# addtt/ladder-vae-pytorch

Measured on AMD Instinct MI355X. Metric: training images/sec (ELBO step: fwd+bwd+Adamax), higher is better.
Workload: dtype f32; 1 GPU; CIFAR10-shaped 15-layer LVAE (BASELINE configs[2]): 32x32x3, zdims 32x15, 4 blocks/layer, 64 filters, gated+skip, DMoL-10, dropout 0.2, free bits 1.0; batch_per_gpu=256, global_batch=256, parallelism=dp1, hip_graph=True

## Files before the change

### include/lvae_hip.h

```cpp
#ifndef LVAE_HIP_H
#define LVAE_HIP_H

#include <stddef.h>
#include <stdint.h>

#ifdef __cplusplus
extern "C" {
#endif

#define LVAE_ABI_VERSION 17

#define LVAE_EINVAL (-1)
#define LVAE_EALIGN (-2)
#define LVAE_EWORKSPACE (-3)

enum { LVAE_STATS_BN_FWD = 0, LVAE_STATS_BN_BWD = 1 };
enum { LVAE_PREC_F32 = 0, LVAE_PREC_BF16 = 1 };
enum { LVAE_DT_F32 = 0, LVAE_DT_BF16 = 1 };
enum {
  LVAE_FORM_AUTO = 0,
  LVAE_FORM_F32_MFMA = 1,
  LVAE_FORM_SIX_PRODUCT = 2,
  LVAE_FORM_SIX_PRODUCT_DIRECT = 3
};
enum { LVAE_ACT_NONE = 0, LVAE_ACT_ELU = 1, LVAE_ACT_RELU = 2, LVAE_ACT_LEAKYRELU = 3, LVAE_ACT_SELU = 4 };

enum {
  LVAE_GATHER_CONV = 0,
  LVAE_GATHER_TRANSPOSED = 1
};

int lvae_abi_version(void);
const char* lvae_last_error(void);

typedef struct lvae_bn_fold {
  const float* parts;
  int32_t rows;
  int64_t M;
  const float* gamma;
  const float* beta;
  float eps, momentum;
  float* running_mean;
  float* running_var;
  float* coef_out;
} lvae_bn_fold;

typedef struct lvae_conv_desc {
  const float* x;
  const float* x2;
  int32_t C1, C2;
  const float* w;
  int64_t w_stap, w_sk, w_sn;
  const float* bias;
  const float* in_scale;
  const float* in_shift;
  int32_t in_act;
  const float* out_scale;
  int32_t out_act;
  float* y;
  int32_t N, H, W, OH, OW, Cout;
  int32_t KH, KW, stride, pad;
  int32_t gather;
  int32_t precision;
  void* workspace;
  int64_t workspace_bytes;
  int32_t workspace_ready;
  float* stats_out;
  const float* stats_pivot;
  int32_t stats_mode;
  int32_t stats_act;
  const float* stats_x;
  const struct lvae_bn_fold* in_fold;
  int32_t form;
  uint8_t x_dtype;
  uint8_t y_dtype;
  uint8_t stats_x_dtype;
  uint8_t reserved_;
} lvae_conv_desc;

size_t lvae_conv2d_workspace(const lvae_conv_desc* d);
int lvae_conv2d_f32(const lvae_conv_desc* d, void* stream);
int lvae_conv1x1_dgrad_cat_f32(const lvae_conv_desc* d, float* dx2, int32_t split, void* stream);
int32_t lvae_conv1x1_dgrad_cat_ok(const lvae_conv_desc* d, int32_t split);
enum {
  LVAE_VARIANT_DIRECT = 0,
  LVAE_VARIANT_POS = 2,
  LVAE_VARIANT_WINO_F32 = 3,
  LVAE_VARIANT_WINO_SIX = 4,
  LVAE_VARIANT_BF16_DIRECT = 5,
  LVAE_VARIANT_SIX_DIRECT = 6
};
int32_t lvae_conv2d_variant(const lvae_conv_desc* d);
int32_t lvae_resblock_bf16_storage(const lvae_conv_desc* d);
int lvae_conv2d_bf16(const lvae_conv_desc* d, void* stream);
int32_t lvae_conv2d_stats_rows(const lvae_conv_desc* d);
int32_t lvae_conv2d_folds_bn_finalize(const lvae_conv_desc* d);
int32_t lvae_conv2d_stats_buffer_rows(const lvae_conv_desc* d);

size_t lvae_conv2d_prepare_entry_bytes(void);
int lvae_conv2d_prepare_entry(const lvae_conv_desc* d, void* entry);
int lvae_conv2d_prepare_weights(const void* entries, int32_t n, int32_t max_cout, void* stream);

int lvae_conv1x1_gate_f32(const lvae_conv_desc* d, const float* res, int32_t act, float* out, void* stream);
int32_t lvae_conv1x1_gate_stats_rows(const lvae_conv_desc* d);
enum {
  LVAE_GATE_PERSISTENT = 1,
  LVAE_GATE_SINGLE_SHOT = 2
};
int32_t lvae_conv1x1_gate_variant(const lvae_conv_desc* d);
int lvae_conv1x1_gate_bwd_f32(const lvae_conv_desc* d, const float* dout, const float* ab, int32_t act, float* dab,
                              void* stream);
int32_t lvae_conv1x1_gate_bwd_ok(const lvae_conv_desc* d);

typedef struct lvae_bn_apply {
  const float* parts;
  int32_t rows;
  int32_t act;
  int64_t M;
  const float* coef;
  const float* dh;
  const float* x;
  const float* add;
  float* dgamma;
  float* dbeta;
  float* out;
  int32_t dh_bf16;
  int32_t reserved_;
  const float* drop;
} lvae_bn_apply;
size_t lvae_conv1x1_gate_bwd_wgrad_workspace(const lvae_conv_desc* d);
int32_t lvae_conv1x1_gate_bwd_wgrad_apply_ok(const lvae_conv_desc* d);
int lvae_conv1x1_gate_bwd_wgrad_f32(const lvae_conv_desc* d, const float* dout, const float* ab, const float* y, int32_t act,
                                    float* dw, int64_t dw_sk, int64_t dw_sn, float* db, void* workspace, size_t workspace_bytes,
                                    const lvae_bn_apply* ap, void* stream);

enum { LVAE_RB_PRO_AFFINE = 0, LVAE_RB_PRO_BN_APPLY = 1, LVAE_RB_PRO_GATE_BWD = 2 };
enum { LVAE_RB_EPI_PLAIN = 0, LVAE_RB_EPI_GATE = 1 };
typedef struct lvae_rb_ext {
  int32_t prologue, epilogue;
  const float* gate_w;
  int64_t gate_w_sk, gate_w_sn;
  void* gate_ws;
  int64_t gate_ws_bytes;
  int32_t gate_ws_ready;
  const float* gate_bias;
  int32_t act;
  const float* res;
  float* ab;
  float* out;
  float* out_stats;
  const float* out_stats_pivot;
  const float* dout;
  const float* ab_in;
  float* dab;
  const float* bwd_parts;
  int32_t bwd_rows;
  int32_t bwd_act;
  int64_t bwd_M;
  const float* bwd_coef;
  const float* bwd_x;
  float* dgamma;
  float* dbeta;
  const float* pro_drop;
  float* xt_out;
  const void* pf_ptr[2];
  int64_t pf_bytes[2];
  const float* ap_parts;
  int32_t ap_rows;
  int32_t ap_act;
  int64_t ap_M;
  const float* ap_coef;
  const float* ap_dh;
  const float* ap_x;
  const float* ap_add;
  float* ap_dgamma;
  float* ap_dbeta;
  float* ap_out;
} lvae_rb_ext;
size_t lvae_resblock_gate_workspace(const lvae_conv_desc* g);
int lvae_resblock_gate_prepare_entry(const lvae_conv_desc* g, void* entry);
int32_t lvae_resblock_conv_rows(const lvae_conv_desc* d);
int32_t lvae_resblock_conv_gate_rows(const lvae_conv_desc* d);
size_t lvae_resblock_conv_workspace(const lvae_conv_desc* d);
int lvae_resblock_conv_prepare_entry(const lvae_conv_desc* d, void* entry);
int lvae_resblock_conv_f32(const lvae_conv_desc* d, const lvae_rb_ext* ext, void* stream);

size_t lvae_conv2d_wgrad_workspace(const lvae_conv_desc* d);
int lvae_conv2d_wgrad_f32(const lvae_conv_desc* d, const float* dy, float* dw, float* db, void* workspace,
                          size_t workspace_bytes, void* stream);
int lvae_conv2d_wgrad_bf16(const lvae_conv_desc* d, const float* dy, float* dw, float* db, void* workspace, size_t workspace_bytes,
                           void* stream);
int32_t lvae_conv2d_wgrad_apply_ok(const lvae_conv_desc* d);
int lvae_conv2d_wgrad_apply_f32(const lvae_conv_desc* d, const lvae_bn_apply* ap, float* dw, float* db, void* workspace,
                                size_t workspace_bytes, void* stream);
enum {
  LVAE_WGRAD_VARIANT_GENERIC = 0,
  LVAE_WGRAD_VARIANT_IMG = 1,
  LVAE_WGRAD_VARIANT_BF16 = 2,
  LVAE_WGRAD_VARIANT_WINO = 3,
  LVAE_WGRAD_VARIANT_DIRECT_1X1 = 4,
  LVAE_WGRAD_VARIANT_TILE = 5,
  LVAE_WGRAD_VARIANT_THIN = 6
};
int32_t lvae_conv2d_wgrad_variant(const lvae_conv_desc* d);
size_t lvae_conv2d_wgrad_grouped_workspace(const lvae_conv_desc* descs, int32_t n);
int lvae_conv2d_wgrad_grouped_f32(const lvae_conv_desc* descs, const float* const* dy, float* const* dw, float* const* db,
                                  int32_t n, void* workspace, size_t workspace_bytes, void* stream);
int32_t lvae_conv2d_wgrad_grouped_schedule(const lvae_conv_desc* descs, int32_t n, int32_t* launch_of);

size_t lvae_bn_stats_workspace(int64_t M, int32_t C);
int lvae_bn_stats_f32(const float* x, int64_t M, int32_t C, const float* gamma, const float* beta, float eps,
                      float momentum, float* running_mean, float* running_var, float* scale, float* shift,
                      float* mean, float* rstd, void* workspace, size_t workspace_bytes, void* stream);
int lvae_bn_finalize_parts_f32(const float* parts, int32_t rows, int64_t M, int32_t C, const float* pivot, const float* gamma,
                               const float* beta, float eps, float momentum, float* running_mean, float* running_var,
                               float* scale, float* shift, float* mean, float* rstd, void* stream);
int lvae_bn_eval_coeffs_f32(int32_t C, const float* gamma, const float* beta, const float* running_mean,
                            const float* running_var, float eps, float* scale, float* shift, void* stream);

int lvae_affine_act_f32(const float* x, int64_t M, int32_t C, const float* scale, const float* shift, int32_t act,
                        const float* row_scale, int64_t rows_per_n, float* y, void* stream);

int lvae_affine_act_bwd_f32(const float* dh, const float* x, int64_t M, int32_t C, const float* scale,
                            const float* shift, int32_t act, int32_t bn_train, const float* mean, const float* rstd,
                            float* dgamma, float* dbeta, const float* drop, int64_t rows_per_n, const float* add,
                            float* dx, void* workspace, size_t workspace_bytes, void* stream);
int lvae_affine_act_bwd_parts_f32(const float* parts, int32_t rows, const float* dh, const float* x, int64_t M, int32_t C,
                                  const float* scale, const float* shift, int32_t act, const float* mean, const float* rstd,
                                  float* dgamma, float* dbeta, const float* drop, int64_t rows_per_n, const float* add,
                                  float* dx, void* workspace, size_t workspace_bytes, int32_t dtypes, void* stream);

int lvae_gate_fwd_f32(const float* ab, const float* res, int64_t M, int32_t C, int32_t act, float* out, void* stream);
int lvae_gate_bwd_f32(const float* dout, const float* ab, int64_t M, int32_t C, int32_t act, float* dab, void* stream);

int lvae_act_bwd_from_out_f32(const float* dy, const float* y, int64_t n, int32_t act, float* dx, void* stream);
int lvae_add_f32(const float* a, const float* b, int64_t n, float* out, void* stream);
int lvae_add3_f32(const float* a, const float* b, const float* c, int64_t n, float* out, void* stream);
int lvae_sum_of_row_means_f32(const float* x, int32_t L, int32_t N, float* out, void* stream);
int lvae_scale_rows_add_f32(const float* a, const float* row_scale, int64_t rows_per_n, int32_t C, const float* b,
                            int64_t M, float* out, void* stream);
int lvae_colsum_f32(const float* x, int64_t R, int64_t P, float* out, int32_t accumulate, void* stream);

int lvae_normal_stochastic_fwd_f32(const float* p, int32_t p_bcast, const float* q, const float* eps, int32_t N,
                                   int32_t HW, int32_t Z, int32_t mode, int32_t analytical_kl, float* z,
                                   float* logprob_p, float* logprob_q, float* kl_samplewise, float* kl_spatial,
// ... 121 lines not shown
```

### ladder-vae-pytorch_amd/_C.py

```python
import ctypes as C
import os

import torch

_HERE = os.path.dirname(os.path.abspath(__file__))
LIB_PATH = os.path.join(_HERE, 'liblvae_hip.so')

ACT = {None: 0, 'none': 0, 'elu': 1, 'relu': 2, 'leakyrelu': 3, 'selu': 4}
GATHER_CONV, GATHER_TRANSPOSED = 0, 1
PREC_F32, PREC_BF16 = 0, 1
DT_F32, DT_BF16 = 0, 1
VARIANT_DIRECT, VARIANT_POS, VARIANT_WINO_F32, VARIANT_WINO_SIX, VARIANT_BF16_DIRECT, VARIANT_SIX_DIRECT = 0, 2, 3, 4, 5, 6
GATE_PERSISTENT, GATE_SINGLE_SHOT = 1, 2
WGRAD_VARIANT_GENERIC, WGRAD_VARIANT_IMG, WGRAD_VARIANT_BF16, WGRAD_VARIANT_WINO, WGRAD_VARIANT_DIRECT_1X1, WGRAD_VARIANT_TILE, WGRAD_VARIANT_THIN = range(7)
FEED_U8, FEED_F32 = 0, 1
FORM_AUTO, FORM_F32_MFMA, FORM_SIX_PRODUCT, FORM_SIX_PRODUCT_DIRECT = 0, 1, 2, 3


class LvaeHipError(RuntimeError):
    pass


class ConvDesc(C.Structure):
    _fields_ = [
        ('x', C.c_void_p), ('x2', C.c_void_p), ('C1', C.c_int32), ('C2', C.c_int32),
        ('w', C.c_void_p), ('w_stap', C.c_int64), ('w_sk', C.c_int64), ('w_sn', C.c_int64),
        ('bias', C.c_void_p), ('in_scale', C.c_void_p), ('in_shift', C.c_void_p), ('in_act', C.c_int32),
        ('out_scale', C.c_void_p), ('out_act', C.c_int32), ('y', C.c_void_p),
        ('N', C.c_int32), ('H', C.c_int32), ('W', C.c_int32), ('OH', C.c_int32), ('OW', C.c_int32),
        ('Cout', C.c_int32), ('KH', C.c_int32), ('KW', C.c_int32), ('stride', C.c_int32), ('pad', C.c_int32),
        ('gather', C.c_int32), ('precision', C.c_int32), ('workspace', C.c_void_p), ('workspace_bytes', C.c_int64), ('workspace_ready', C.c_int32), ('stats_out', C.c_void_p), ('stats_pivot', C.c_void_p), ('stats_mode', C.c_int32), ('stats_act', C.c_int32),
        ('stats_x', C.c_void_p),
        ('in_fold', C.c_void_p),
        ('form', C.c_int32), ('x_dtype', C.c_uint8), ('y_dtype', C.c_uint8), ('stats_x_dtype', C.c_uint8), ('reserved_', C.c_uint8),
    ]


class BnFold(C.Structure):
    _fields_ = [('parts', C.c_void_p), ('rows', C.c_int32), ('M', C.c_int64), ('gamma', C.c_void_p), ('beta', C.c_void_p),
                ('eps', C.c_float), ('momentum', C.c_float), ('running_mean', C.c_void_p), ('running_var', C.c_void_p),
                ('coef_out', C.c_void_p)]


class BnApply(C.Structure):
    _fields_ = [('parts', C.c_void_p), ('rows', C.c_int32), ('act', C.c_int32), ('M', C.c_int64), ('coef', C.c_void_p), ('dh', C.c_void_p),
                ('x', C.c_void_p), ('add', C.c_void_p), ('dgamma', C.c_void_p), ('dbeta', C.c_void_p), ('out', C.c_void_p),
                ('dh_bf16', C.c_int32), ('reserved_', C.c_int32), ('drop', C.c_void_p)]


class RbExt(C.Structure):
    _fields_ = [('prologue', C.c_int32), ('epilogue', C.c_int32), ('gate_w', C.c_void_p), ('gate_w_sk', C.c_int64), ('gate_w_sn', C.c_int64),
                ('gate_ws', C.c_void_p), ('gate_ws_bytes', C.c_int64), ('gate_ws_ready', C.c_int32), ('gate_bias', C.c_void_p), ('act', C.c_int32), ('res', C.c_void_p), ('ab', C.c_void_p), ('out', C.c_void_p),
                ('out_stats', C.c_void_p), ('out_stats_pivot', C.c_void_p), ('dout', C.c_void_p), ('ab_in', C.c_void_p), ('dab', C.c_void_p),
                ('bwd_parts', C.c_void_p), ('bwd_rows', C.c_int32), ('bwd_act', C.c_int32), ('bwd_M', C.c_int64), ('bwd_coef', C.c_void_p),
                ('bwd_x', C.c_void_p), ('dgamma', C.c_void_p), ('dbeta', C.c_void_p), ('pro_drop', C.c_void_p), ('xt_out', C.c_void_p),
                ('pf_ptr', C.c_void_p * 2), ('pf_bytes', C.c_int64 * 2),
                ('ap_parts', C.c_void_p), ('ap_rows', C.c_int32), ('ap_act', C.c_int32), ('ap_M', C.c_int64), ('ap_coef', C.c_void_p),
                ('ap_dh', C.c_void_p), ('ap_x', C.c_void_p), ('ap_add', C.c_void_p), ('ap_dgamma', C.c_void_p), ('ap_dbeta', C.c_void_p),
                ('ap_out', C.c_void_p)]


class LrScheduleStruct(C.Structure):
    _fields_ = [('base_lr', C.c_float), ('min_lr', C.c_float), ('gamma', C.c_float), ('kind', C.c_int32),
                ('warmup_steps', C.c_int64), ('decay_steps', C.c_int64)]


LR_KINDS = {'constant': 0, 'cosine': 1, 'linear': 2, 'step': 3, 'exp': 4}

RB_PRO_AFFINE, RB_PRO_BN_APPLY, RB_PRO_GATE_BWD = 0, 1, 2
RB_EPI_PLAIN, RB_EPI_GATE = 0, 1

ABI_VERSION = 17

_P, _I, _L, _F, _Z, _U = C.c_void_p, C.c_int32, C.c_int64, C.c_float, C.c_size_t, C.c_uint64

SIGNATURES = {
    'lvae_abi_version': (C.c_int, []),
    'lvae_last_error': (C.c_char_p, []),
    'lvae_conv2d_workspace': (_Z, [C.POINTER(ConvDesc)]),
    'lvae_conv2d_f32': (C.c_int, [C.POINTER(ConvDesc), _P]),
    'lvae_conv2d_bf16': (C.c_int, [C.POINTER(ConvDesc), _P]),
    'lvae_conv1x1_dgrad_cat_f32': (C.c_int, [C.POINTER(ConvDesc), _P, _I, _P]),
    'lvae_conv1x1_dgrad_cat_ok': (_I, [C.POINTER(ConvDesc), _I]),
    'lvae_conv2d_stats_rows': (_I, [C.POINTER(ConvDesc)]),
    'lvae_conv2d_variant': (_I, [C.POINTER(ConvDesc)]),
    'lvae_resblock_bf16_storage': (_I, [C.POINTER(ConvDesc)]),
    'lvae_conv2d_folds_bn_finalize': (_I, [C.POINTER(ConvDesc)]),
    'lvae_conv2d_stats_buffer_rows': (_I, [C.POINTER(ConvDesc)]),
    'lvae_conv2d_prepare_entry_bytes': (_Z, []),
    'lvae_conv2d_prepare_entry': (C.c_int, [C.POINTER(ConvDesc), _P]),
    'lvae_conv2d_prepare_weights': (C.c_int, [_P, _I, _I, _P]),
    'lvae_conv1x1_gate_f32': (C.c_int, [C.POINTER(ConvDesc), _P, _I, _P, _P]),
    'lvae_conv1x1_gate_stats_rows': (_I, [C.POINTER(ConvDesc)]),
    'lvae_conv1x1_gate_variant': (_I, [C.POINTER(ConvDesc)]),
    'lvae_conv1x1_gate_bwd_f32': (C.c_int, [C.POINTER(ConvDesc), _P, _P, _I, _P, _P]),
    'lvae_conv1x1_gate_bwd_ok': (_I, [C.POINTER(ConvDesc)]),
    'lvae_conv1x1_gate_bwd_wgrad_workspace': (_Z, [C.POINTER(ConvDesc)]),
    'lvae_conv1x1_gate_bwd_wgrad_apply_ok': (_I, [C.POINTER(ConvDesc)]),
    'lvae_conv1x1_gate_bwd_wgrad_f32': (C.c_int, [C.POINTER(ConvDesc), _P, _P, _P, _I, _P, _L, _L, _P, _P, _Z, C.POINTER(BnApply), _P]),
    'lvae_resblock_gate_workspace': (_Z, [C.POINTER(ConvDesc)]),
    'lvae_resblock_gate_prepare_entry': (C.c_int, [C.POINTER(ConvDesc), _P]),
    'lvae_resblock_conv_rows': (_I, [C.POINTER(ConvDesc)]),
    'lvae_resblock_conv_gate_rows': (_I, [C.POINTER(ConvDesc)]),
    'lvae_resblock_conv_workspace': (_Z, [C.POINTER(ConvDesc)]),
    'lvae_resblock_conv_prepare_entry': (C.c_int, [C.POINTER(ConvDesc), _P]),
    'lvae_resblock_conv_f32': (C.c_int, [C.POINTER(ConvDesc), C.POINTER(RbExt), _P]),
    'lvae_conv2d_wgrad_workspace': (_Z, [C.POINTER(ConvDesc)]),
    'lvae_conv2d_wgrad_f32': (C.c_int, [C.POINTER(ConvDesc), _P, _P, _P, _P, _Z, _P]),
    'lvae_conv2d_wgrad_bf16': (C.c_int, [C.POINTER(ConvDesc), _P, _P, _P, _P, _Z, _P]),
    'lvae_conv2d_wgrad_variant': (_I, [C.POINTER(ConvDesc)]),
    'lvae_conv2d_wgrad_apply_ok': (_I, [C.POINTER(ConvDesc)]),
    'lvae_conv2d_wgrad_apply_f32': (C.c_int, [C.POINTER(ConvDesc), C.POINTER(BnApply), _P, _P, _P, _Z, _P]),
    'lvae_conv2d_wgrad_grouped_workspace': (_Z, [C.POINTER(ConvDesc), _I]),
    'lvae_conv2d_wgrad_grouped_f32': (C.c_int, [C.POINTER(ConvDesc), _P, _P, _P, _I, _P, _Z, _P]),
    'lvae_conv2d_wgrad_grouped_schedule': (_I, [C.POINTER(ConvDesc), _I, C.POINTER(_I)]),
    'lvae_bn_stats_workspace': (_Z, [_L, _I]),
    'lvae_bn_stats_f32': (C.c_int, [_P, _L, _I, _P, _P, _F, _F, _P, _P, _P, _P, _P, _P, _P, _Z, _P]),
    'lvae_bn_finalize_parts_f32': (C.c_int, [_P, _I, _L, _I, _P, _P, _P, _F, _F, _P, _P, _P, _P, _P, _P, _P]),
    'lvae_bn_eval_coeffs_f32': (C.c_int, [_I, _P, _P, _P, _P, _F, _P, _P, _P]),
    'lvae_affine_act_f32': (C.c_int, [_P, _L, _I, _P, _P, _I, _P, _L, _P, _P]),
    'lvae_affine_act_bwd_f32': (C.c_int, [_P, _P, _L, _I, _P, _P, _I, _I, _P, _P, _P, _P, _P, _L, _P, _P, _P, _Z, _P]),
    'lvae_affine_act_bwd_parts_f32': (C.c_int, [_P, _I, _P, _P, _L, _I, _P, _P, _I, _P, _P, _P, _P, _P, _L, _P, _P, _P, _Z, _I, _P]),
    'lvae_gate_fwd_f32': (C.c_int, [_P, _P, _L, _I, _I, _P, _P]),
    'lvae_gate_bwd_f32': (C.c_int, [_P, _P, _L, _I, _I, _P, _P]),
    'lvae_act_bwd_from_out_f32': (C.c_int, [_P, _P, _L, _I, _P, _P]),
    'lvae_add_f32': (C.c_int, [_P, _P, _L, _P, _P]),
    'lvae_add3_f32': (C.c_int, [_P, _P, _P, _L, _P, _P]),
    'lvae_sum_of_row_means_f32': (C.c_int, [_P, _I, _I, _P, _P]),
    'lvae_scale_rows_add_f32': (C.c_int, [_P, _P, _L, _I, _P, _L, _P, _P]),
    'lvae_colsum_f32': (C.c_int, [_P, _L, _L, _P, _I, _P]),
    'lvae_normal_stochastic_fwd_f32': (C.c_int, [_P, _I, _P, _P, _I, _I, _I, _I, _I, _P, _P, _P, _P, _P, _P]),
    'lvae_normal_stochastic_bwd_f32': (C.c_int, [_P, _I, _P, _P, _P, _P, _P, _P, _P, _P, _I, _I, _I, _I, _I, _P, _P, _P]),
    'lvae_normal_prior_sample_f32': (C.c_int, [_P, _I, _P, _F, _P, _I, _I, _I, _P, _P, _P]),
    'lvae_kl_elementwise_fwd_f32': (C.c_int, [_P, _I, _P, _I, _P, _I, _I, _I, _I, _P, _P]),
    'lvae_kl_elementwise_bwd_f32': (C.c_int, [_P, _I, _P, _I, _P, _P, _I, _I, _I, _I, _P, _P, _P, _P]),
    'lvae_bernoulli_fwd_f32': (C.c_int, [_P, _P, _P, _I, _L, _P, _P, _P, _P, _P, _P]),
    'lvae_dmol_workspace': (_Z, [_I, _I]),
    'lvae_dmol_ll_fwd_f32': (C.c_int, [_P, _P, _I, _I, _I, _P, _P, _P, _Z, _P]),
    'lvae_dmol_sample_f32': (C.c_int, [_P, _P, _P, _I, _I, _I, _P, _P]),
    'lvae_gaussian_fwd_f32': (C.c_int, [_P, _P, _P, _I, _L, _I, _P, _P, _P, _P]),
    'lvae_discr_logistic_fwd_f32': (C.c_int, [_P, _P, _P, _I, _L, _I, _P, _P, _P, _P, _P, _P]),
    'lvae_scale_per_sample_f32': (C.c_int, [_P, _P, _I, _L, _P, _P]),
    'lvae_upsample2x_fwd_f32': (C.c_int, [_P, _I, _I, _I, _I, _P, _P]),
    'lvae_upsample2x_bwd_f32': (C.c_int, [_P, _I, _I, _I, _I, _P, _P]),
    'lvae_pad_crop_f32': (C.c_int, [_P, _I, _I, _I, _I, _I, _P, _I, _I, _I, _P]),
    'lvae_kl_bookkeeping_fwd_f32': (C.c_int, [_P, _I, _I, _F, _P, _P, _P, _P]),
    'lvae_kl_bookkeeping_bwd_f32': (C.c_int, [_P, _I, _I, _F, _P, _P, _P, _P, _P]),
    'lvae_elbo_loss_fwd_f32': (C.c_int, [_P, _P, _P, _F, _I, _P, _P, _P]),
    'lvae_elbo_loss_bwd_f32': (C.c_int, [_P, _F, _I, _P, _P, _P]),
    'lvae_elbo_loss_fwd_anneal_f32': (C.c_int, [_P, _P, _P, _P, _L, _I, _P, _P, _P]),
    'lvae_elbo_loss_bwd_anneal_f32': (C.c_int, [_P, _P, _L, _I, _P, _P, _P]),
    'lvae_iw_loss_fwd_f32': (C.c_int, [_P, _P, _F, _I, _I, _P, _P, _P, _P, _P]),
    'lvae_iw_loss_bwd_f32': (C.c_int, [_P, _P, _F, _I, _I, _P, _P, _P]),
    'lvae_iw_loss_fwd_anneal_f32': (C.c_int, [_P, _P, _P, _L, _I, _I, _P, _P, _P, _P, _P]),
    'lvae_iw_loss_bwd_anneal_f32': (C.c_int, [_P, _P, _P, _L, _I, _I, _P, _P, _P]),
    'lvae_repeat_samples_fwd_f32': (C.c_int, [_P, _L, _I, _P, _P]),
    'lvae_repeat_samples_bwd_f32': (C.c_int, [_P, _L, _I, _P, _P]),
    'lvae_iw_online_f32': (C.c_int, [_P, _P, _I, _I, _I, _P, _P, _P]),
    'lvae_eval_online_f32': (C.c_int, [_P, _P, _P, _P, _P, _I, _I, _I, _P]),
    'lvae_eval_totals_f64': (C.c_int, [_P, _I, _I, _I, _P, _P]),
    'lvae_latent_stats_workspace': (_Z, [_I, _I, _I]),
    'lvae_latent_stats_fold_f32': (C.c_int, [_P, _I, _P, _I, _I, _I, _P, _P, _Z, _P]),
    'lvae_latent_stats_finalize_f64': (C.c_int, [_P, _L, _L, C.c_double, C.c_double, _P, _P, _P]),
    'lvae_summary_fold_f64': (C.c_int, [_P, _P, _P, _P, _P, _P, _P, _P, _I, _P, _P]),
    'lvae_summary_take_f64': (C.c_int, [_P, _I, _P, _P]),
    'lvae_image_border_count_f32': (C.c_int, [_P, _I, _P, _I, _I, _I, _I, _I, _F, _P, _P]),
    'lvae_image_grid_u8': (C.c_int, [_P, _I, _P, _I, _I, _I, _I, _I, _I, _P, _F, _P, _L, _P]),
    'lvae_batch_gather_f32': (C.c_int, [_P, _I, _I, _I, _I, _I, _I, _P, _P, _I, _I, _I, _L, _I, _P, _P]),
    'lvae_iw_logmeanexp_f32': (C.c_int, [_P, _I, _I, _P, _P]),
    'lvae_adamax_step_f32': (C.c_int, [_P, _P, _P, _P, _P, _L, _F, _F, _F, _F, _F, _P, _P, _P]),
    'lvae_adamax_ema_step_f32': (C.c_int, [_P, _P, _P, _P, _P, _L, _F, _F, _F, _F, _F, _P, _P, _P, _F, _P]),
    'lvae_lr_schedule_at': (C.c_int, [C.POINTER(LrScheduleStruct), _U, C.POINTER(C.c_float)]),
    'lvae_adamax_sched_step_f32': (C.c_int, [_P, _P, _P, _P, _P, _L, C.POINTER(LrScheduleStruct), _F, _F, _F, _F, _P, _P, _P, _F, _P, _P]),
    'lvae_swap_f32': (C.c_int, [_P, _P, _L, _P]),
    'lvae_sumsq_workspace': (_Z, [_L]),
    'lvae_l2norm_f32': (C.c_int, [_P, _L, _P, _P, _Z, _P]),
    'lvae_rng_fill_f32': (C.c_int, [_P, _L, _I, _F, _F, _U, _P, _U, _P]),
    'lvae_counter_advance': (C.c_int, [_P, _U, _P]),
    'lvae_fill_f32': (C.c_int, [_P, _L, _F, _P]),
    'lvae_allreduce_unique_id': (C.c_int, [C.c_char_p, _P]),
    'lvae_allreduce_init': (C.c_int, [C.c_char_p, _P, _I, _I, C.POINTER(C.c_void_p)]),
    'lvae_allreduce_enqueue': (C.c_int, [_P, _P, _L, _P, _P, _P]),
    'lvae_allreduce_wait': (C.c_int, [_P, _P, _P]),
    'lvae_allreduce_destroy': (C.c_int, [_P]),
}

_lib = None


def load():
    global _lib
    if _lib is not None:
        return _lib
    if not os.path.exists(LIB_PATH):
        raise LvaeHipError("%s is missing: build it with `python -c 'import __graft_entry__ as g; g.build()'` or "
                           "`make -C ladder-vae-pytorch_amd/csrc`. There is no CPU / PyTorch fallback." % LIB_PATH)
    lib = C.CDLL(LIB_PATH)
    for name, (res, args) in SIGNATURES.items():
        fn = getattr(lib, name)
        fn.restype, fn.argtypes = res, args
    if lib.lvae_abi_version() != ABI_VERSION:
        raise LvaeHipError("liblvae_hip.so ABI version %d, expected %d" % (lib.lvae_abi_version(), ABI_VERSION))
    _lib = lib
    return lib


def stream_ptr():
    return torch.cuda.current_stream().cuda_stream


def ptr(t, dtypes=(torch.float32, torch.int64, torch.uint8)):
    if t is None:
        return None
    if not t.is_cuda:
        raise LvaeHipError("lvae_hip kernels need CUDA/HIP tensors; got a %s tensor (no CPU fallback exists)" % t.device)
    if t.dtype not in dtypes:
        raise LvaeHipError("unexpected dtype %s for this entry point (it has no storage-type argument for this tensor)" % t.dtype)
    return t.data_ptr()


def ptr_dt(t):
    return ptr(t, (torch.float32, torch.bfloat16))


def check(rc, name):
    if rc != 0:
        raise LvaeHipError("%s failed (%d): %s" % (name, rc, load().lvae_last_error().decode()))


def call(name, *args):
    check(getattr(load(), name)(*args), name)
```

### ladder-vae-pytorch_amd/csrc/conv_igemm.hip

```cpp
#include <stdlib.h>

#include "lvae_host.h"

namespace lvae {

constexpr int KC = 32;
constexpr int LDK = KC + 4;

enum { B_NCONTIG = 0, B_KCONTIG = 1, B_SCALAR = 2 };

struct ConvArgs {
  lvae_conv_desc d;
  int M;
  int ohw;
  int Cin;
  int nchunks;
  int cpt;
  int ktot;
  int ntn;
};

__device__ __forceinline__ bool tap_coord(int o, int k, int stride, int pad, int limit, int gather, int& i) {
  if (gather == LVAE_GATHER_CONV) {
    i = o * stride - pad + k;
// ... 142 lines not shown
        f32x4 v = {0.f, 0.f, 0.f, 0.f};
        if (k < a.Cin && n < d.Cout)
          v = *reinterpret_cast<const f32x4*>(d.w + tap * d.w_stap + (int64_t)n * d.w_sn + k);
        b_reg[p] = v;
      }
    } else {
      int tap, k;
      bool k_ok;
      if (A_VEC) {
        tap = chunk / a.cpt;
        k = (chunk - tap * a.cpt) * KC + (t & 31);
        k_ok = k < a.Cin;
      } else {
        const int kf = chunk * KC + (t & 31);
        k_ok = kf < a.ktot;
        tap = k_ok ? kf / a.Cin : 0;
        k = kf - tap * a.Cin;
      }
#pragma unroll
      for (int e = 0; e < BS; ++e) {
        const int n = n0 + (t >> 5) + 8 * e;
        b_sreg[e] = (k_ok && n < d.Cout) ? d.w[tap * d.w_stap + (int64_t)k * d.w_sk + (int64_t)n * d.w_sn] : 0.f;
      }
    }
  };

  auto store_stage = [&](int buf) {
    float* Ab = As + buf * BM * LDK;
    float* Bb = Bs + buf * BN * LDK;
    if (A_VEC) {
#pragma unroll
      for (int p = 0; p < AP; ++p) *reinterpret_cast<f32x4*>(Ab + (arow + 32 * p) * LDK + ac4) = a_reg[p];
    } else {
#pragma unroll
      for (int e = 0; e < AS; ++e) Ab[((t >> 5) + 8 * e) * LDK + (t & 31)] = a_sreg[e];
    }
    if (B_MODE == B_NCONTIG) {
      constexpr int F4 = BN / 4;
#pragma unroll
      for (int p = 0; p < BP; ++p) {
        const int idx = t + 256 * p, kk = idx / F4, nl = (idx - kk * F4) * 4;
#pragma unroll
        for (int j = 0; j < 4; ++j) Bb[(nl + j) * LDK + kk] = b_reg[p][j];
      }
    } else if (B_MODE == B_KCONTIG) {
#pragma unroll
      for (int p = 0; p < BP; ++p)
        *reinterpret_cast<f32x4*>(Bb + ((t >> 3) + 32 * p) * LDK + (t & 7) * 4) = b_reg[p];
    } else {
#pragma unroll
      for (int e = 0; e < BS; ++e) Bb[((t >> 5) + 8 * e) * LDK + (t & 31)] = b_sreg[e];
    }
  };

  f32x16 acc[MI][NI];
#pragma unroll
  for (int mi = 0; mi < MI; ++mi)
#pragma unroll
    for (int ni = 0; ni < NI; ++ni)
#pragma unroll
      for (int r = 0; r < 16; ++r) acc[mi][ni][r] = 0.f;

  load_stage(0);
  store_stage(0);
  __syncthreads();

  for (int c = 0; c < a.nchunks; ++c) {
    const int buf = c & 1;
    if (c + 1 < a.nchunks) load_stage(c + 1);
    const float* Ab = As + buf * BM * LDK + (wm * WM + li) * LDK + 4 * lh;
    const float* Bb = Bs + buf * BN * LDK + (wn * WN + li) * LDK + 4 * lh;
#pragma unroll
    for (int kk = 0; kk < KC; kk += 8) {
      f32x4 af[MI], bf[NI];
#pragma unroll
      for (int mi = 0; mi < MI; ++mi) af[mi] = *reinterpret_cast<const f32x4*>(Ab + mi * 32 * LDK + kk);
#pragma unroll
      for (int ni = 0; ni < NI; ++ni) bf[ni] = *reinterpret_cast<const f32x4*>(Bb + ni * 32 * LDK + kk);
#pragma unroll
      for (int j = 0; j < 4; ++j)
#pragma unroll
        for (int mi = 0; mi < MI; ++mi)
#pragma unroll
          for (int ni = 0; ni < NI; ++ni)
            acc[mi][ni] = __builtin_amdgcn_mfma_f32_32x32x2f32(af[mi][j], bf[ni][j], acc[mi][ni], 0, 0, 0);
    }
    if (c + 1 < a.nchunks) store_stage(buf ^ 1);
    __syncthreads();
  }

#pragma unroll
  for (int ni = 0; ni < NI; ++ni) {
    const int col = n0 + wn * WN + ni * 32 + li;
    if (col >= d.Cout) continue;
    const float bias = d.bias ? d.bias[col] : 0.f;
#pragma unroll
    for (int mi = 0; mi < MI; ++mi) {
#pragma unroll
      for (int r = 0; r < 16; ++r) {
        const int row = m0 + wm * WM + mi * 32 + (r & 3) + 8 * (r >> 2) + 4 * lh;
        if (row >= a.M) continue;
        float v = acc[mi][ni][r] + bias;
        if (d.out_scale) v *= d.out_scale[(size_t)(row / a.ohw) * d.Cout + col];
        v = act_fwd(v, d.out_act);
        d.y[(size_t)row * d.Cout + col] = v;
      }
    }
  }
}

template <int BM, int BN, bool A_VEC, int B_MODE>
static int launch_conv(const ConvArgs& a, hipStream_t s) {
  constexpr size_t smem = (size_t)(2 * BM * LDK + 2 * BN * LDK) * sizeof(float);
  const int ntm = (a.M + BM - 1) / BM;
  ConvArgs b = a;
  b.ntn = (a.d.Cout + BN - 1) / BN;
  return launch_lds<conv_igemm_kernel<BM, BN, A_VEC, B_MODE>>("conv2d", dim3(ntm * b.ntn), dim3(256), smem, (int)smem, s, b);
}

template <bool A_VEC, int B_MODE>
static int dispatch_tile(const ConvArgs& a, hipStream_t s) {
  const bool wide = a.d.Cout > 64;
  const int ntn128 = wide ? (a.d.Cout + 127) / 128 : 1;
  const bool big = (int64_t)((a.M + 127) / 128) * ntn128 >= 256;
  if (wide) return big ? launch_conv<128, 128, A_VEC, B_MODE>(a, s) : launch_conv<64, 128, A_VEC, B_MODE>(a, s);
  return big ? launch_conv<128, 64, A_VEC, B_MODE>(a, s) : launch_conv<64, 64, A_VEC, B_MODE>(a, s);
}

int conv_desc_check(const lvae_conv_desc* d, const char* who) {
  LVAE_REQUIRE(d != nullptr, LVAE_EINVAL, "%s: null descriptor", who);
  LVAE_REQUIRE(d->x && d->w, LVAE_EINVAL, "%s: null x or w", who);
  LVAE_REQUIRE(d->N > 0 && d->H > 0 && d->W > 0 && d->OH > 0 && d->OW > 0 && d->Cout > 0 && d->C1 > 0 && d->C2 >= 0,
               LVAE_EINVAL, "%s: non-positive dimension", who);
  LVAE_REQUIRE((d->C2 == 0) == (d->x2 == nullptr), LVAE_EINVAL, "%s: x2/C2 mismatch", who);
  LVAE_REQUIRE(d->KH > 0 && d->KW > 0 && d->stride > 0 && d->pad >= 0, LVAE_EINVAL, "%s: bad kernel geometry", who);
  LVAE_REQUIRE(d->gather == LVAE_GATHER_CONV || d->gather == LVAE_GATHER_TRANSPOSED, LVAE_EINVAL, "%s: bad gather", who);
  LVAE_REQUIRE((d->in_scale == nullptr) || (d->in_shift != nullptr), LVAE_EINVAL, "%s: in_scale without in_shift", who);
  LVAE_REQUIRE((int64_t)d->N * d->OH * d->OW < (int64_t)1 << 31 && (int64_t)d->N * d->H * d->W < (int64_t)1 << 31,
               LVAE_EINVAL, "%s: pixel count exceeds int32", who);
  if (d->gather == LVAE_GATHER_CONV) {
    LVAE_REQUIRE((d->H + 2 * d->pad - d->KH) / d->stride + 1 == d->OH && (d->W + 2 * d->pad - d->KW) / d->stride + 1 == d->OW,
                 LVAE_EINVAL, "%s: output size %dx%d inconsistent with input %dx%d k%d s%d p%d", who, d->OH, d->OW, d->H,
                 d->W, d->KH, d->stride, d->pad);
  } else {
    LVAE_REQUIRE((d->OH + 2 * d->pad - d->KH) / d->stride + 1 == d->H && (d->OW + 2 * d->pad - d->KW) / d->stride + 1 == d->W,
                 LVAE_EINVAL, "%s: transposed geometry inconsistent (in %dx%d out %dx%d k%d s%d p%d)", who, d->H, d->W,
                 d->OH, d->OW, d->KH, d->stride, d->pad);
  }
  return 0;
}

static bool aligned16(const void* p) { return (reinterpret_cast<uintptr_t>(p) & 15) == 0; }

enum { ROUTE_POS, ROUTE_BF16, ROUTE_WINO, ROUTE_HALO, ROUTE_1X1, ROUTE_GENERIC };

struct ConvRoute {
  int kind = ROUTE_GENERIC;
  ConvPlan plan;
};

static ConvRoute conv_route(const lvae_conv_desc* d, bool assume_ws = false) {
  static const bool halo_off = tune("LVAE_DISABLE_HALO", 0) != 0;
  lvae_conv_desc t = *d;
  t.in_fold = nullptr;
  ConvRoute r;
  if (halo_off) return r;
  if (conv3x3_pos_plan(&t, r.plan)) r.kind = ROUTE_POS;
  else if (conv3x3_bf16_plan(&t, assume_ws, r.plan)) r.kind = ROUTE_BF16;
  else if (conv3x3_wino_plan(&t, assume_ws, r.plan)) r.kind = ROUTE_WINO;
  else if (conv3x3_halo_plan(&t, r.plan)) r.kind = ROUTE_HALO;
  else if (conv1x1_plan(&t, PwForm{}, r.plan)) r.kind = ROUTE_1X1;
  return r;
}

}

using namespace lvae;

extern "C" size_t lvae_conv2d_workspace(const lvae_conv_desc* d) { return d ? conv_route(d, true).plan.workspace : 0; }

extern "C" int32_t lvae_conv2d_variant(const lvae_conv_desc* d) { return d ? conv_route(d).plan.variant : LVAE_VARIANT_DIRECT; }

extern "C" int32_t lvae_resblock_bf16_storage(const lvae_conv_desc* d) {
  if (d == nullptr || d->precision != LVAE_PREC_BF16 || d->C1 != 64 || d->C2 != 0 || d->Cout != 64 || d->gather != LVAE_GATHER_CONV) return 0;
  const ConvPlan f = conv_route(d).plan;
  if (f.variant != LVAE_VARIANT_BF16_DIRECT || f.rows <= 0) return 0;
  lvae_conv_desc t = *d;
  t.gather = LVAE_GATHER_TRANSPOSED;
  const ConvPlan b = conv_route(&t).plan;
  if (b.variant != LVAE_VARIANT_BF16_DIRECT || b.rows <= 0) return 0;
  WgradPlan wp;
  if (!conv3x3_wgrad_bf16_plan(d, wp)) return 0;
  lvae_conv_desc g = *d;
  g.KH = g.KW = 1; g.pad = 0; g.Cout = 128; g.in_scale = g.in_shift = nullptr; g.out_scale = nullptr; g.in_act = g.out_act = 0; g.in_fold = nullptr;
  ConvPlan gp;
  if (!conv1x1_gate_fwd_plan(&g, gp)) return 0;
  g.C1 = 128; g.Cout = 64; g.w_sk = 1; g.w_sn = 128;
  return conv1x1_gate_bwd_fused_plan(&g, false, gp) ? 1 : 0;
}

extern "C" int32_t lvae_conv2d_stats_rows(const lvae_conv_desc* d) { return d ? conv_route(d).plan.rows : 0; }

extern "C" int32_t lvae_conv2d_folds_bn_finalize(const lvae_conv_desc* d) { return d && conv_route(d).plan.folds ? 1 : 0; }

extern "C" int32_t lvae_conv2d_stats_buffer_rows(const lvae_conv_desc* d) {
  if (d == nullptr) return 0;
  const ConvPlan p = conv_route(d).plan;
  if (p.rows <= 0) return 0;
  if (d->stats_mode != LVAE_STATS_BN_FWD) return p.rows;
  return p.rows + (p.folds ? 1 : 0);
}

extern "C" int lvae_conv2d_f32(const lvae_conv_desc* d, void* stream) {
  int rc = conv_desc_check(d, "lvae_conv2d_f32");
  if (rc) return rc;
  LVAE_REQUIRE(d->y != nullptr, LVAE_EINVAL, "lvae_conv2d_f32: null y");
  const ConvRoute r = conv_route(d);
  LVAE_REQUIRE(d->stats_out == nullptr || (d->stats_pivot != nullptr && r.plan.rows > 0), LVAE_EINVAL,
               "lvae_conv2d_f32: stats_out set but lvae_conv2d_stats_rows(d) == 0 (this kernel variant has no statistics epilogue)");
  LVAE_REQUIRE(d->stats_out == nullptr || d->stats_mode == LVAE_STATS_BN_FWD ||
                   (d->stats_mode == LVAE_STATS_BN_BWD && d->stats_x != nullptr && (reinterpret_cast<uintptr_t>(d->stats_x) & 15) == 0),
               LVAE_EINVAL, "lvae_conv2d_f32: bad stats_mode / stats_x");
  LVAE_REQUIRE((d->x_dtype == LVAE_DT_F32 && d->y_dtype == LVAE_DT_F32 && d->stats_x_dtype == LVAE_DT_F32) ||
                   r.plan.variant == LVAE_VARIANT_BF16_DIRECT,
               LVAE_EINVAL, "lvae_conv2d_f32: bf16-stored tensors need the bf16 3x3 kernel (precision LVAE_PREC_BF16, lvae_conv2d_variant(d) == "
                            "LVAE_VARIANT_BF16_DIRECT)");
  LVAE_REQUIRE(d->in_fold == nullptr || (r.plan.folds && d->in_fold->parts != nullptr && (reinterpret_cast<uintptr_t>(d->in_fold->parts) & 15) == 0 &&
                                         d->C1 % 4 == 0 && d->in_fold->rows > 0 && d->in_fold->M > 0 && d->in_scale == nullptr),
               LVAE_EINVAL,
               "lvae_conv2d_f32: in_fold set but lvae_conv2d_folds_bn_finalize(d) == 0 (or bad parts / rows / M, or in_scale given too)");
  hipStream_t s = (hipStream_t)stream;
  switch (r.kind) {
    case ROUTE_POS: return conv3x3_pos_launch(d, s);
    case ROUTE_BF16: return conv3x3_bf16_launch(d, r.plan, s);
    case ROUTE_WINO: return conv3x3_wino_launch(d, s);
    case ROUTE_HALO: return conv3x3_halo_launch(d, s);
    case ROUTE_1X1: return conv1x1_launch(d, PwForm{}, s);
  }
  ConvArgs a;
  a.d = *d;
  a.M = d->N * d->OH * d->OW;
  a.ohw = d->OH * d->OW;
  a.Cin = d->C1 + d->C2;
  a.ktot = d->KH * d->KW * a.Cin;
  a.ntn = 1;
  const bool a_vec = (d->C1 % 4 == 0) && (d->C2 % 4 == 0) && aligned16(d->x) && (!d->x2 || aligned16(d->x2)) &&
                     (!d->in_scale || (aligned16(d->in_scale) && aligned16(d->in_shift)));
  if (a_vec) {
    a.cpt = (a.Cin + KC - 1) / KC;
    a.nchunks = d->KH * d->KW * a.cpt;
  } else {
    a.cpt = 1;
    a.nchunks = (a.ktot + KC - 1) / KC;
  }
  const bool w16 = aligned16(d->w) && (d->w_stap % 4 == 0);
  if (!a_vec) return dispatch_tile<false, B_SCALAR>(a, s);
  if (d->w_sn == 1 && w16 && d->Cout % 4 == 0 && d->w_sk % 4 == 0) return dispatch_tile<true, B_NCONTIG>(a, s);
  if (d->w_sk == 1 && w16 && a.Cin % 4 == 0 && d->w_sn % 4 == 0) return dispatch_tile<true, B_KCONTIG>(a, s);
  return dispatch_tile<true, B_SCALAR>(a, s);
}

extern "C" int lvae_conv2d_bf16(const lvae_conv_desc* d, void* stream) {
  LVAE_REQUIRE(d != nullptr, LVAE_EINVAL, "lvae_conv2d_bf16: null descriptor");
  lvae_conv_desc dd = *d;
  dd.precision = LVAE_PREC_BF16;
  return lvae_conv2d_f32(&dd, stream);
}
```

### ladder-vae-pytorch_amd/csrc/lvae_host.h

```cpp
#pragma once
#include "lvae_common.h"

namespace lvae {

struct ConvPlan {
  int32_t variant = LVAE_VARIANT_DIRECT;
  int32_t rows = 0;
  bool folds = false;
  size_t workspace = 0;
};

struct ReduceArgs {
  const float* slab_w;
  const float* slab_b;
  int ksplit, ntaps, Cin, Cout;
  int64_t stap, sk, sn;
  float* dw;
  float* db;
};
constexpr int kMaxReduceGroup = 12;

struct WgradPlan {
  int32_t variant = LVAE_WGRAD_VARIANT_GENERIC;
  int32_t group = -1;
  int32_t slabs = 0;
  size_t w_floats = 0, b_floats = 0;
  size_t workspace = 0;
  bool takes_bf16_storage = false, apply_ok = false;
  void set_slabs(int n, size_t w, size_t b) { slabs = n, w_floats = w, b_floats = b, workspace = (size_t)n * (w + b) * sizeof(float); }
};

struct WgradOp {
  const lvae_conv_desc* d;
  WgradPlan plan;
  const float* dy;
  float *dw, *db;
  void* workspace;
  float* slab_w() const { return static_cast<float*>(workspace); }
  float* slab_b() const { return db ? slab_w() + (size_t)plan.slabs * plan.w_floats : nullptr; }
};
constexpr int kWgradTileGroup = 12, kWgradWinoGroup = 12, kWgradImgGroup = 32;

int conv_desc_check(const lvae_conv_desc* d, const char* who);

bool conv3x3_halo_plan(const lvae_conv_desc* d, ConvPlan& p);
int conv3x3_halo_launch(const lvae_conv_desc* d, hipStream_t s);

bool conv3x3_pos_plan(const lvae_conv_desc* d, ConvPlan& p);
int conv3x3_pos_launch(const lvae_conv_desc* d, hipStream_t s);

bool conv3x3_wino_plan(const lvae_conv_desc* d, bool assume_ws, ConvPlan& p);
int conv3x3_wino_launch(const lvae_conv_desc* d, hipStream_t s);
int conv3x3_wino2_gate_rows(const lvae_conv_desc* d);
int conv3x3_wino2_gate_launch(const lvae_conv_desc* d, const lvae_rb_ext* gate, hipStream_t s);

int conv3x3_bf16_form(const lvae_conv_desc* d);
bool conv3x3_bf16_plan(const lvae_conv_desc* d, bool assume_ws, ConvPlan& p);
int conv3x3_bf16_launch(const lvae_conv_desc* d, const ConvPlan& p, hipStream_t s);
size_t conv3x3_bf16_workspace(const lvae_conv_desc* d, int split);
void conv3x3_bf16_prep_entry(const lvae_conv_desc* d, int split, void* entry);
int conv3x3_bf16_prepare_single(const lvae_conv_desc* d, int split, hipStream_t s);
int conv3x3_bf16_prepare_batched(const void* entries, int n, int npad, hipStream_t s);
size_t resblock_gate_ws_bytes(const lvae_conv_desc* d, int planes);
void resblock_gate_prep_entry(const lvae_conv_desc* d, int planes, void* entry);
int resblock_gate_prepare_single(const lvae_conv_desc* d, int planes, hipStream_t s);
bool conv3x3_wgrad_bf16_plan(const lvae_conv_desc* d, WgradPlan& p);
int conv3x3_wgrad_bf16_launch(const WgradOp& o, hipStream_t s);

enum { PW_PLAIN, PW_GATE_FWD, PW_GATE_BWD, PW_DGRAD_CAT };
struct PwForm {
  int kind = PW_PLAIN;
  int act = 0;
  const float* res = nullptr;
  float* out = nullptr;
  const float* dout = nullptr;
  const float* ab = nullptr;
  float* dab = nullptr;
  float* y2 = nullptr;
  int split = 0;
};
bool conv1x1_plan(const lvae_conv_desc* d, const PwForm& f, ConvPlan& p);
int conv1x1_launch(const lvae_conv_desc* d, const PwForm& f, hipStream_t s);

bool conv1x1_gate_fwd_plan(const lvae_conv_desc* d, ConvPlan& p);
int conv1x1_gate_fwd_launch(const lvae_conv_desc* d, const ConvPlan& p, const float* res, float* out, int act, hipStream_t s);

bool conv1x1_gate_bwd_fused_plan(const lvae_conv_desc* d, bool with_apply, ConvPlan& p);

void wgrad_reduce_launch(const float* slab_w, const float* slab_b, int ksplit, int ntaps, int Cin, int Cout, int64_t stap,
                         int64_t sk, int64_t sn, float* dw, float* db, hipStream_t s);
void wgrad_reduce_grouped_launch(const ReduceArgs* r, int n, hipStream_t s);
int wgrad_op_reduce(const WgradOp& o, hipStream_t s);

bool conv_wgrad_img_plan(const lvae_conv_desc* d, WgradPlan& p);
int conv_wgrad_img_grouped(const WgradOp* o, int n, hipStream_t s);

bool conv_wgrad_tile_plan(const lvae_conv_desc* d, WgradPlan& p);
int conv_wgrad_tile_launch(const WgradOp* o, int n, hipStream_t s);

bool conv_wgrad_wino_plan(const lvae_conv_desc* d, WgradPlan& p);
int conv_wgrad_wino_launch(const WgradOp* o, int n, hipStream_t s);
int conv_wgrad_wino_apply_launch(const WgradOp& o, const lvae_bn_apply* ap, hipStream_t s);

bool conv1x1_wgrad_plan(const lvae_conv_desc* d, WgradPlan& p);
int conv1x1_wgrad_launch(const WgradOp& o, hipStream_t s);

template <auto Kern, typename Args>
int launch_lds(const char* name, dim3 grid, dim3 block, size_t lds, int max_lds, hipStream_t s, const Args& a) {
  static std::atomic<bool> attr_set{false};
  if (!attr_set) {
    hipError_t e = hipFuncSetAttribute(reinterpret_cast<const void*>(Kern), hipFuncAttributeMaxDynamicSharedMemorySize, max_lds);
    if (e != hipSuccess) {
      set_error("%s: hipFuncSetAttribute failed: %s", name, hipGetErrorString(e));
      return (int)e;
    }
    attr_set = true;
  }
  hipLaunchKernelGGL(Kern, grid, block, lds, s, a);
  LVAE_LAUNCH_CHECK(name);
  return 0;
}

}
```

Measured before the change: 8817 images/s.

## Add position-major MFMA kernel for stride-2 and transposed 3x3 resample convs

Adds a dedicated kernel for 3x3 stride-2 convolutions and their transposed form (downsample/upsample layers) with Cin up to 64. Each block owns one output position, 32 batch rows and 32 output channels, stages only the valid taps in LDS, and accumulates with f32 MFMA, fusing the input BN/activation prologue and the bias/scale/activation epilogue. It is routed ahead of the generic implicit-GEMM fallback and exposed through a new position_major query. This replaces the generic kernel for the resampling layers, at the cost of one block per output position and large per-block LDS use.

```diff
diff --git a/include/lvae_hip.h b/include/lvae_hip.h
--- a/include/lvae_hip.h
+++ b/include/lvae_hip.h
@@ -91,6 +91,7 @@
   LVAE_VARIANT_SIX_DIRECT = 6
 };
 int32_t lvae_conv2d_variant(const lvae_conv_desc* d);
+int32_t lvae_conv2d_position_major(const lvae_conv_desc* d);
 int32_t lvae_resblock_bf16_storage(const lvae_conv_desc* d);
 int lvae_conv2d_bf16(const lvae_conv_desc* d, void* stream);
 int32_t lvae_conv2d_stats_rows(const lvae_conv_desc* d);
diff --git a/ladder-vae-pytorch_amd/_C.py b/ladder-vae-pytorch_amd/_C.py
--- a/ladder-vae-pytorch_amd/_C.py
+++ b/ladder-vae-pytorch_amd/_C.py
@@ -84,6 +84,7 @@
     'lvae_conv1x1_dgrad_cat_ok': (_I, [C.POINTER(ConvDesc), _I]),
     'lvae_conv2d_stats_rows': (_I, [C.POINTER(ConvDesc)]),
     'lvae_conv2d_variant': (_I, [C.POINTER(ConvDesc)]),
+    'lvae_conv2d_position_major': (_I, [C.POINTER(ConvDesc)]),
     'lvae_resblock_bf16_storage': (_I, [C.POINTER(ConvDesc)]),
     'lvae_conv2d_folds_bn_finalize': (_I, [C.POINTER(ConvDesc)]),
     'lvae_conv2d_stats_buffer_rows': (_I, [C.POINTER(ConvDesc)]),
diff --git a/ladder-vae-pytorch_amd/csrc/conv3x3_resample.hip b/ladder-vae-pytorch_amd/csrc/conv3x3_resample.hip
--- /dev/null
+++ b/ladder-vae-pytorch_amd/csrc/conv3x3_resample.hip
@@ -0,0 +1,224 @@
+#include "lvae_host.h"
+
+namespace lvae {
+
+struct ResampleArgs {
+  lvae_conv_desc d;
+  int P, Cin, n_groups, ntn;
+  uint32_t m_ow;
+};
+
+template <bool TRANSPOSED>
+__device__ __forceinline__ bool resample_tap(int o, int j, int limit, int& k, int& i) {
+  if (!TRANSPOSED) {
+    k = j;
+    i = 2 * o - 1 + j;
+    return (unsigned)i < (unsigned)limit;
+  }
+  const bool odd = (o & 1) != 0;
+  k = odd ? 2 * j : 1;
+  i = (o + 1 - k) >> 1;
+  return (odd || j == 0) && i < limit;
+}
+
+template <int CIN_T, bool B_KCONTIG, bool TRANSPOSED>
+__global__ __launch_bounds__(256) void conv3x3_resample_kernel(ResampleArgs a) {
+  kernarg_warmup<(sizeof(ResampleArgs) < 1024 ? sizeof(ResampleArgs) : 1024)>();
+  constexpr int NT = TRANSPOSED ? 2 : 3;
+  constexpr int MAXT = NT * NT;
+  constexpr int LDA = CIN_T + 4;
+  constexpr int CIN4 = CIN_T / 4;
+  constexpr int RPP = 256 / CIN4;
+  constexpr int APT = 32 / RPP;
+  constexpr int ASZ = 32 * LDA;
+  constexpr int BSZ = B_KCONTIG ? 32 * LDA : CIN_T * 32;
+  constexpr int BPT = CIN_T * 32 / 4 / 256;
+  constexpr int KW_ = CIN_T / 4;
+  extern __shared__ __attribute__((aligned(16))) float smem[];
+  const lvae_conv_desc& d = a.d;
+  const int t = threadIdx.x, lane = t & 63, wave = t >> 6, li = lane & 31, lh = lane >> 5;
+
+  const int bid = blockIdx.x;
+  const int tile_n = bid % a.ntn, rest = bid / a.ntn;
+  const int pos = rest % a.P, ig = rest / a.P;
+  const int oy = fastdiv(pos, a.m_ow), ox = pos - oy * d.OW;
+  const int n0 = ig * 32, co0 = tile_n * 32;
+  const int Cin = a.Cin;
+  const int nrows = min(32, d.N - n0);
+
+  f32x4 av[MAXT][APT], bv[MAXT][BPT];
+  const int c4 = (t % CIN4) * 4, r0 = t / CIN4;
+  const bool c_ok = c4 < Cin;
+  unsigned valid = 0;
+#pragma unroll
+  for (int c = 0; c < MAXT; ++c) {
+    int kh, kw, iy, ix;
+    const bool vy = resample_tap<TRANSPOSED>(oy, c / NT, d.H, kh, iy);
+    const bool vx = resample_tap<TRANSPOSED>(ox, c % NT, d.W, kw, ix);
+    if (!(vy && vx)) continue;
+    valid |= 1u << c;
+#pragma unroll
+    for (int p = 0; p < APT; ++p) {
+      const int r = r0 + p * RPP;
+      const bool ok = (r < nrows) & c_ok;
+      const size_t off = ok ? ((size_t)((n0 + r) * d.H + iy) * d.W + ix) * Cin + c4 : 0;
+      av[c][p] = *reinterpret_cast<const f32x4*>(d.x + off);
+    }
+    const float* wt = d.w + (int64_t)(kh * 3 + kw) * d.w_stap;
+#pragma unroll
+    for (int p = 0; p < BPT; ++p) {
+      const int idx = t + 256 * p;
+      f32x4 v = {0.f, 0.f, 0.f, 0.f};
+      if (B_KCONTIG) {
+        const int n = idx / CIN4, k = (idx - n * CIN4) * 4;
+        if (co0 + n < d.Cout && k < Cin) v = *reinterpret_cast<const f32x4*>(wt + (int64_t)(co0 + n) * d.w_sn + k);
+      } else {
+        const int k = idx >> 3, n = (idx & 7) * 4;
+        if (k < Cin && co0 + n < d.Cout) v = *reinterpret_cast<const f32x4*>(wt + (int64_t)k * d.w_sk + co0 + n);
+      }
+      bv[c][p] = v;
+    }
+  }
+
+  f32x4 sc = {1.f, 1.f, 1.f, 1.f}, sh = {0.f, 0.f, 0.f, 0.f};
+  const bool has_tf = d.in_scale != nullptr;
+  if (has_tf && c_ok) {
+    sc = *reinterpret_cast<const f32x4*>(d.in_scale + c4);
+    sh = *reinterpret_cast<const f32x4*>(d.in_shift + c4);
+  }
+
+  const int ntaps = __popc(valid);
+  float* As = smem;
+  float* Bs = smem + (size_t)ntaps * ASZ;
+  {
+    int slot = 0;
+#pragma unroll
+    for (int c = 0; c < MAXT; ++c) {
+      if (!((valid >> c) & 1u)) continue;
+#pragma unroll
+      for (int p = 0; p < APT; ++p) {
+        const int r = r0 + p * RPP;
+        f32x4 v = {0.f, 0.f, 0.f, 0.f};
+        if ((r < nrows) & c_ok) {
+          v = av[c][p];
+          if (has_tf) v = act_fwd4(v * sc + sh, d.in_act);
+        }
+        *reinterpret_cast<f32x4*>(As + slot * ASZ + r * LDA + c4) = v;
+      }
+#pragma unroll
+      for (int p = 0; p < BPT; ++p) {
+        const int idx = t + 256 * p;
+        if (B_KCONTIG) {
+          const int n = idx / CIN4, k = (idx - n * CIN4) * 4;
+          *reinterpret_cast<f32x4*>(Bs + slot * BSZ + n * LDA + k) = bv[c][p];
+        } else {
+          const int k = idx >> 3, n = (idx & 7) * 4;
+          *reinterpret_cast<f32x4*>(Bs + slot * BSZ + k * 32 + n) = bv[c][p];
+        }
+      }
+      ++slot;
+    }
+  }
+  __syncthreads();
+
+  f32x16 acc;
+#pragma unroll
+  for (int r = 0; r < 16; ++r) acc[r] = 0.f;
+  const int kb = wave * KW_;
+  for (int slot = 0; slot < ntaps; ++slot) {
+    const float* Ab = As + slot * ASZ + li * LDA + kb + 4 * lh;
+    const float* Bb = Bs + slot * BSZ;
+#pragma unroll
+    for (int q = 0; q < KW_ / 8; ++q) {
+      const f32x4 af = *reinterpret_cast<const f32x4*>(Ab + q * 8);
+      f32x4 bf;
+      if (B_KCONTIG) {
+        bf = *reinterpret_cast<const f32x4*>(Bb + li * LDA + kb + q * 8 + 4 * lh);
+      } else {
+#pragma unroll
+        for (int j = 0; j < 4; ++j) bf[j] = Bb[(kb + q * 8 + 4 * lh + j) * 32 + li];
+      }
+#pragma unroll
+      for (int j = 0; j < 4; ++j) acc = __builtin_amdgcn_mfma_f32_32x32x2f32(af[j], bf[j], acc, 0, 0, 0);
+    }
+  }
+  __syncthreads();
+
+  constexpr int LDO = 36;
+  float* Os = smem;
+#pragma unroll
+  for (int r = 0; r < 16; ++r) Os[wave * 32 * LDO + ((r & 3) + 8 * (r >> 2) + 4 * lh) * LDO + li] = acc[r];
+  __syncthreads();
+
+  const int row = t >> 3, oc4 = (t & 7) * 4, col = co0 + oc4;
+  if (row < nrows && col < d.Cout) {
+    f32x4 v = *reinterpret_cast<const f32x4*>(Os + row * LDO + oc4);
+#pragma unroll
+    for (int w = 1; w < 4; ++w) v += *reinterpret_cast<const f32x4*>(Os + w * 32 * LDO + row * LDO + oc4);
+    if (d.bias) v += *reinterpret_cast<const f32x4*>(d.bias + col);
+    const int n = n0 + row;
+    if (d.out_scale) v = v * *reinterpret_cast<const f32x4*>(d.out_scale + (size_t)n * d.Cout + col);
+    v = act_fwd4(v, d.out_act);
+    const size_t o = ((size_t)(n * d.OH + oy) * d.OW + ox) * d.Cout + col;
+    *reinterpret_cast<f32x4*>(d.y + o) = v;
+  }
+}
+
+static bool resample_select(const lvae_conv_desc* d, bool& ncontig) {
+  static const bool off = tune("LVAE_DISABLE_RESAMPLE", 0) != 0;
+  if (off) return false;
+  const int Cin = d->C1;
+  if (d->KH != 3 || d->KW != 3 || d->stride != 2 || d->pad != 1 || d->x2 != nullptr || d->C2 != 0) return false;
+  if (d->gather != LVAE_GATHER_CONV && d->gather != LVAE_GATHER_TRANSPOSED) return false;
+  if (d->x_dtype != LVAE_DT_F32 || d->y_dtype != LVAE_DT_F32) return false;
+  if (Cin > 64 || Cin % 4 != 0 || d->Cout % 4 != 0 || d->w_stap % 4 != 0) return false;
+  if (!al16_or_null(d->x) || !al16_or_null(d->w) || !al16_or_null(d->y) || !al16_or_null(d->bias) || !al16_or_null(d->out_scale) || !al16_or_null(d->in_scale) ||
+      !al16_or_null(d->in_shift))
+    return false;
+  const bool kc = d->w_sk == 1 && d->w_sn % 4 == 0, nc = d->w_sn == 1 && d->w_sk % 4 == 0;
+  if (!kc && !nc) return false;
+  if (d->gather == LVAE_GATHER_CONV && (int64_t)((d->N + 31) / 32) * d->OH * d->OW * ((d->Cout + 31) / 32) > 1024) return false;
+  ncontig = nc;
+  return true;
+}
+
+bool conv3x3_resample_plan(const lvae_conv_desc* d, ConvPlan& p) {
+  bool ncontig;
+  if (!resample_select(d, ncontig)) return false;
+  p = ConvPlan{};
+  return true;
+}
+
+template <int CIN_T, bool KC, bool TR>
+static int launch_resample(const ResampleArgs& a, hipStream_t s) {
+  constexpr int nt = TR ? 2 : 3;
+  const int th = a.d.H >= nt ? nt : a.d.H, tw = a.d.W >= nt ? nt : a.d.W;
+  constexpr size_t asz = (size_t)32 * (CIN_T + 4), bsz = KC ? (size_t)32 * (CIN_T + 4) : (size_t)CIN_T * 32;
+  size_t lds = (size_t)th * tw * (asz + bsz) * sizeof(float);
+  const size_t lds_out = (size_t)4 * 32 * 36 * sizeof(float);
+  if (lds < lds_out) lds = lds_out;
+  return launch_lds<conv3x3_resample_kernel<CIN_T, KC, TR>>("conv3x3_resample", dim3(a.n_groups * a.P * a.ntn), dim3(256), lds, 157 * 1024, s, a);
+}
+
+template <int CIN_T, bool KC>
+static int launch_resample_gather(const ResampleArgs& a, hipStream_t s) {
+  return a.d.gather == LVAE_GATHER_TRANSPOSED ? launch_resample<CIN_T, KC, true>(a, s) : launch_resample<CIN_T, KC, false>(a, s);
+}
+
+int conv3x3_resample_launch(const lvae_conv_desc* d, hipStream_t s) {
+  bool ncontig = false;
+  resample_select(d, ncontig);
+  ResampleArgs a;
+  a.d = *d;
+  a.d.in_fold = nullptr;
+  a.P = d->OH * d->OW;
+  a.Cin = d->C1;
+  a.n_groups = (d->N + 31) / 32;
+  a.ntn = (d->Cout + 31) / 32;
+  a.m_ow = fastdiv_magic(d->OW);
+  const bool kc = !ncontig;
+  if (d->C1 <= 32) return kc ? launch_resample_gather<32, true>(a, s) : launch_resample_gather<32, false>(a, s);
+  return kc ? launch_resample_gather<64, true>(a, s) : launch_resample_gather<64, false>(a, s);
+}
+
+}
diff --git a/ladder-vae-pytorch_amd/csrc/conv_igemm.hip b/ladder-vae-pytorch_amd/csrc/conv_igemm.hip
--- a/ladder-vae-pytorch_amd/csrc/conv_igemm.hip
+++ b/ladder-vae-pytorch_amd/csrc/conv_igemm.hip
@@ -318,7 +318,7 @@
 
 static bool aligned16(const void* p) { return (reinterpret_cast<uintptr_t>(p) & 15) == 0; }
 
-enum { ROUTE_POS, ROUTE_BF16, ROUTE_WINO, ROUTE_HALO, ROUTE_1X1, ROUTE_GENERIC };
+enum { ROUTE_POS, ROUTE_BF16, ROUTE_WINO, ROUTE_HALO, ROUTE_1X1, ROUTE_RESAMPLE, ROUTE_GENERIC };
 
 struct ConvRoute {
   int kind = ROUTE_GENERIC;
@@ -336,6 +336,7 @@
   else if (conv3x3_wino_plan(&t, assume_ws, r.plan)) r.kind = ROUTE_WINO;
   else if (conv3x3_halo_plan(&t, r.plan)) r.kind = ROUTE_HALO;
   else if (conv1x1_plan(&t, PwForm{}, r.plan)) r.kind = ROUTE_1X1;
+  else if (conv3x3_resample_plan(&t, r.plan)) r.kind = ROUTE_RESAMPLE;
   return r;
 }
 
@@ -346,6 +347,12 @@
 extern "C" size_t lvae_conv2d_workspace(const lvae_conv_desc* d) { return d ? conv_route(d, true).plan.workspace : 0; }
 
 extern "C" int32_t lvae_conv2d_variant(const lvae_conv_desc* d) { return d ? conv_route(d).plan.variant : LVAE_VARIANT_DIRECT; }
+
+extern "C" int32_t lvae_conv2d_position_major(const lvae_conv_desc* d) {
+  if (d == nullptr) return 0;
+  const int kind = conv_route(d).kind;
+  return kind == ROUTE_POS || kind == ROUTE_RESAMPLE ? 1 : 0;
+}
 
 extern "C" int32_t lvae_resblock_bf16_storage(const lvae_conv_desc* d) {
   if (d == nullptr || d->precision != LVAE_PREC_BF16 || d->C1 != 64 || d->C2 != 0 || d->Cout != 64 || d->gather != LVAE_GATHER_CONV) return 0;
@@ -402,6 +409,7 @@
     case ROUTE_WINO: return conv3x3_wino_launch(d, s);
     case ROUTE_HALO: return conv3x3_halo_launch(d, s);
     case ROUTE_1X1: return conv1x1_launch(d, PwForm{}, s);
+    case ROUTE_RESAMPLE: return conv3x3_resample_launch(d, s);
   }
   ConvArgs a;
   a.d = *d;
diff --git a/ladder-vae-pytorch_amd/csrc/lvae_host.h b/ladder-vae-pytorch_amd/csrc/lvae_host.h
--- a/ladder-vae-pytorch_amd/csrc/lvae_host.h
+++ b/ladder-vae-pytorch_amd/csrc/lvae_host.h
@@ -48,6 +48,9 @@
 
 bool conv3x3_pos_plan(const lvae_conv_desc* d, ConvPlan& p);
 int conv3x3_pos_launch(const lvae_conv_desc* d, hipStream_t s);
+
+bool conv3x3_resample_plan(const lvae_conv_desc* d, ConvPlan& p);
+int conv3x3_resample_launch(const lvae_conv_desc* d, hipStream_t s);
 
 bool conv3x3_wino_plan(const lvae_conv_desc* d, bool assume_ws, ConvPlan& p);
 int conv3x3_wino_launch(const lvae_conv_desc* d, hipStream_t s);
```

Result: faster. 8931 images/s (median of 6 runs) (+1.3%).
